# chrischoy/DeepGlobalRegistration

Measured on AMD Instinct MI355X. Metric: pair registrations/sec (FCGF x2 + 1-NN + 6-D inlier net + gate + weighted Procrustes + SE(3) refinement), higher is better.
Workload: dtype f32 results via 2 x f16 split operands (3 f16 MFMA products per MAC, f32 accumulate); k = 1 convs, kNN re-evaluation and registration in exact f32, SVD in f64

## Files before the change

### deepglobalregistration_amd/_lib.py

```python
import ctypes as C
import os
import threading

import torch

_HERE = os.path.dirname(os.path.abspath(__file__))
LIB_PATH = os.environ.get('DGR_HIP_LIB') or os.path.join(_HERE, 'lib', 'libdgr_hip.so')

DGR_OK, DGR_EINVAL, DGR_EHIP, DGR_ENOMEM, DGR_ESVD, DGR_EINTERNAL = 0, -1, -2, -3, -4, -5
STATUS_OK, STATUS_LOW_CONFIDENCE, STATUS_SVD_FAILED, STATUS_SAFEGUARD = 0, 1, 2, 3
STATUS_FLAG_ICP_SKIPPED, STATUS_MASK = 0x100, 0xff

c_i32p, c_i64p, c_f32p, c_f64p = (C.POINTER(C.c_int32), C.POINTER(C.c_int64),
                                  C.POINTER(C.c_float), C.POINTER(C.c_double))
vp = C.c_void_p


class WeightDesc(C.Structure):
    _fields_ = [('name', C.c_char_p), ('data', vp), ('numel', C.c_int64)]


class Params(C.Structure):
    _fields_ = [('clip_weight_thresh', C.c_float), ('voxel_size', C.c_float),
                ('inlier_feature_type', C.c_int), ('max_iter', C.c_int),
# ... 26 lines not shown
    'dgr_net_get_intermediate': (C.c_int, [vp, vp, C.c_char_p, vp, C.c_int64, c_i64p, c_i64p]),
    'dgr_net_layer_stats': (C.c_int, [vp, vp, C.c_int, c_i64p]),
    'dgr_net_num_layers': (C.c_int, [vp]),
    'dgr_net_rerun_layer': (C.c_int, [vp, vp, C.c_int, C.c_int, c_f32p, c_f32p]),
    'dgr_maps_create': (C.c_int, [vp, vp, C.c_int64, C.c_int, C.c_int, C.POINTER(vp), vp]),
    'dgr_maps_destroy': (None, [vp]),
    'dgr_maps_get_coords': (C.c_int, [vp, C.c_int, vp, C.c_int64, c_i64p]),
    'dgr_maps_get_kernel_map': (C.c_int, [vp, C.c_int, C.c_int, vp, C.c_int64, vp, vp, C.c_int64,
                                          c_i64p, c_i64p]),
    'dgr_knn1_l2': (C.c_int, [vp, vp, C.c_int64, vp, C.c_int64, C.c_int, C.c_int, vp, vp, vp]),
    'dgr_knn1_l2_batch': (C.c_int, [vp, vp, c_i64p, vp, c_i64p, C.c_int, C.c_int, C.c_int, vp, vp, vp]),
    'dgr_knn_l2': (C.c_int, [vp, vp, C.c_int64, vp, C.c_int64, C.c_int, C.c_int, C.c_int, vp, vp, vp]),
    'dgr_knn_l2_batch': (C.c_int, [vp, vp, c_i64p, vp, c_i64p, C.c_int, C.c_int, C.c_int, C.c_int, vp, vp,
                                   vp]),
    'dgr_inlier_inputs': (C.c_int, [vp, vp, vp, C.c_int64, vp, vp, C.c_int64, vp, C.c_int, vp, vp, vp]),
    'dgr_sigmoid_clip_sum': (C.c_int, [vp, vp, C.c_int64, C.c_float, vp, c_f64p, vp]),
    'dgr_gather_rows3': (C.c_int, [vp, vp, vp, C.c_int64, vp, vp]),
    'dgr_weighted_procrustes': (C.c_int, [vp, vp, vp, vp, C.c_int64, C.c_float, c_f32p, c_f32p, vp]),
    'dgr_se3_refine': (C.c_int, [vp, vp, vp, vp, C.c_int64, C.c_float, C.c_int, C.c_int, C.c_double,
                                 c_f32p, c_f32p, c_i32p, c_f32p, c_i32p, vp]),
    'dgr_register_batch': (C.c_int, [vp, vp, vp, vp, vp, c_i64p, vp, vp, c_i64p, C.c_int,
                                     C.POINTER(Params), vp, vp, c_f32p, c_i32p, c_f32p, vp]),
    'dgr_register_pairs': (C.c_int, [vp, vp, vp, vp, vp, c_i64p, C.c_int, C.c_int, c_i32p, C.c_int,
                                     C.POINTER(Params), vp, vp, c_f32p, c_i32p, c_f32p, vp]),
    'dgr_register_batch_f64': (C.c_int, [vp, c_f64p, C.c_int64, c_i64p]),
    'dgr_register_batch_output': (C.c_int, [vp, C.c_int, vp, C.c_int64, c_i64p, vp]),
    'dgr_ctx_set_profiling': (C.c_int, [vp, C.c_int]),
    'dgr_icp_point_to_point': (C.c_int, [vp, vp, C.c_int64, vp, C.c_int64, C.c_double, c_f64p, C.c_int, C.c_double,
                                          C.c_double, c_f64p, c_f64p, vp]),
    'dgr_ransac_correspondence': (C.c_int, [vp, vp, vp, C.c_int64, C.c_double, C.c_int64, C.c_uint32, c_f64p, c_f64p, vp]),
    'dgr_ctx_stage_times': (C.c_int, [vp, c_f32p]),
    'dgr_ctx_stage_times_v2': (C.c_int, [vp, c_f32p, C.c_int, C.POINTER(C.c_int)]),
    'dgr_ctx_conv_launches': (C.c_int64, [vp]),
    'dgr_ctx_conv_launch_times': (C.c_int, [vp, c_f32p, c_f32p, C.c_int64, C.POINTER(C.c_int64)]),
    'dgr_ctx_conv_launch_kernel_us': (C.c_int, [vp, c_f32p, C.c_int64, C.POINTER(C.c_int64)]),
    'dgr_ctx_conv_launch_kinds': (C.c_int, [vp, C.c_char_p, C.c_int64, C.POINTER(C.c_int64)]),
    'dgr_radius_pairs_batch': (C.c_int, [vp, vp, c_i64p, vp, c_i64p, C.c_int, c_f64p, C.c_double, C.c_int, vp, vp,
                                         C.c_int64, c_i64p, vp]),
    'dgr_pairs_isin_batch': (C.c_int, [vp, vp, c_i64p, vp, c_i64p, C.c_int, c_i64p, vp, vp]),
    'dgr_validation_counts': (C.c_int, [vp, vp, vp, C.c_float, c_i64p, C.c_int, c_i64p, vp]),
    'dgr_score_pairs': (C.c_int, [vp, vp, c_i64p, C.c_int, c_i32p, C.c_int, c_f64p, C.c_double, c_f64p, vp]),
    'dgr_pose_graph_optimize': (C.c_int, [vp, C.c_int, c_i64p, c_i64p, c_i32p, c_f64p, c_f64p, C.POINTER(C.c_uint8), c_f64p,
                                          C.POINTER(PgParams), c_f64p, c_f64p, c_f64p, vp]),
    'dgr_voxel_mean': (C.c_int, [vp, vp, C.c_int, c_i64p, C.c_int, c_i32p, C.c_int, c_f64p, c_f64p, C.c_double, vp, vp, vp, vp,
                                 vp, c_i64p, c_i64p, vp]),
    'dgr_tsdf_fragment': (C.c_int, [vp, vp, C.c_int, C.c_int, C.c_int, c_f64p, c_f64p, c_f64p, C.c_double, C.c_double,
                                    C.c_double, C.c_double, C.c_int, C.c_int, C.c_int, vp, C.c_int64, vp, vp, vp, C.c_int64,
                                    c_i64p, c_i64p, c_i64p, vp]),
    'dgr_debug_ortho2rotation': (C.c_int, [vp, vp, C.c_int64, vp, vp, vp, vp]),
    'dgr_debug_se3_refine_from': (C.c_int, [vp, vp, vp, vp, C.c_int64, C.c_float, C.c_int, C.c_int, C.c_double,
                                            c_f64p, c_f64p, vp]),
    'dgr_debug_smooth_l1': (C.c_int, [vp, vp, vp, C.c_int64, C.c_float, vp, vp]),
    'dgr_debug_conv_layer': (C.c_int, [vp, vp, C.c_int, vp, vp, C.c_int, C.c_int64, vp, vp]),
}

_lib = None


def load():
    global _lib
    if _lib is not None:
        return _lib
    if not os.path.exists(LIB_PATH):
        raise RuntimeError(
            f'{LIB_PATH} not found: the HIP extension is not built.  Run '
            '`python -c "import __graft_entry__ as g; g.build()"` (or `make -C '
            'deepglobalregistration_amd/csrc`).  There is no CPU fallback.')
    lib = C.CDLL(LIB_PATH)
    for name, (res, args) in SIGNATURES.items():
        fn = getattr(lib, name)
        fn.restype = res
        fn.argtypes = args
    _lib = lib
    return lib


class DgrError(RuntimeError):
    def __init__(self, code, message):
        super().__init__(f'libdgr_hip error {code}: {message}')
        self.code = code


class DgrInvalidArgument(DgrError, ValueError):

    def __init__(self, message):
        RuntimeError.__init__(self, f'libdgr_hip: {message}')
        self.code = DGR_EINVAL


def check(rc):
    if rc == DGR_OK:
        return
    msg = load().dgr_last_error().decode('utf-8', 'replace')
    if rc == DGR_EINVAL:
        raise DgrInvalidArgument(msg)
    raise DgrError(rc, msg)


_ctxs = {}
_tls = threading.local()


def new_ctx(device):
    lib = load()
    device = torch.device(device)
    idx = device.index if device.index is not None else torch.cuda.current_device()
# ... 40 lines not shown
```

### deepglobalregistration_amd/csrc/conv.hip

```cpp
#include <stdlib.h>

#include <map>

#include "dgr_internal.h"
#include <algorithm>
#include "hash.h"
#include "split.h"

typedef float f32x16 __attribute__((ext_vector_type(16)));
typedef float f32x4 __attribute__((ext_vector_type(4)));
typedef _Float16 f16x4 __attribute__((ext_vector_type(4)));
typedef int i32x4 __attribute__((ext_vector_type(4)));
typedef unsigned int u32x2 __attribute__((ext_vector_type(2)));
typedef unsigned int u32x4 __attribute__((ext_vector_type(4)));

struct ConvKArgs {
  const float *in;
  float *out;
  float *y;
  const float *shift;
  const float *w;
  const int32_t *pair_in, *pair_out, *tile_ptr, *rule_ptr, *n_rows_dev;
  const int4 *tile_desc;
  int in_ld, out_ld, in_relu, y_ld;
// ... 355 lines not shown

template <int CP, int NBLK>
static int launch_identity(const ConvKArgs &ka, int64_t rows_cap, int num_cus, hipStream_t stream) {
  int64_t blocks = std::min<int64_t>((int64_t)num_cus * 4, std::max<int64_t>(1, dgr_ceil_div(rows_cap, 32 * 4 * 2)));
  identity_conv_kernel<CP, NBLK><<<(int)blocks, 256, 0, stream>>>(ka);
  DGR_LAUNCH_CHECK();
  return DGR_OK;
}

int dgr_conv_launch(const DgrConvLaunch &a, int num_cus, hipStream_t stream, const char **kernel_name) {
  ConvKArgs ka;
  ka.in = a.in; ka.out = a.out; ka.w = a.w; ka.y = a.y; ka.shift = a.shift; ka.y_ld = a.cout;
  ka.pair_in = a.pair_in; ka.pair_out = a.pair_out; ka.tile_ptr = a.tile_ptr; ka.rule_ptr = a.rule_ptr;
  ka.n_rows_dev = a.n_rows_dev; ka.tile_desc = a.tile_desc;
  ka.in_ld = a.in_ld; ka.out_ld = a.out_ld; ka.in_relu = a.in_relu;
  ka.cin = a.cin; ka.cin_pad = a.cin_pad; ka.cout = a.cout; ka.K = a.K;
  ka.l2_normalize = a.l2_normalize;
  DGR_REQUIRE(!a.l2_normalize || (a.pair_in == nullptr && a.cout <= 32 && a.cout_pad == 32),
              "fused l2 normalisation needs an identity map and Cout <= 32 (got %d)", a.cout);
  DGR_REQUIRE(a.cin_pad % 8 == 0 && a.cin_pad >= a.cin && a.cin_pad <= 256, "bad cin_pad %d", a.cin_pad);
  const int64_t tile_bound = a.tile_bound > 0 ? a.tile_bound : (int64_t)num_cus * 4;
  const bool vec = ((a.cin | a.in_ld) & 3) == 0;
  if (a.pair_in == nullptr && vec && a.cin == a.cin_pad && a.tile_bound > 0) {
#define DGR_ID(CPV, NBV)                                                                          \
  if (a.cin_pad == CPV && a.cout_pad == 32 * NBV) {                                               \
    if (kernel_name) *kernel_name = "identity_conv_kernel<" #CPV ", " #NBV ">";                   \
    return launch_identity<CPV, NBV>(ka, a.tile_bound * DGR_TILE_M, num_cus, stream);             \
  }
    DGR_ID(64, 1) DGR_ID(64, 2) DGR_ID(96, 2)
#undef DGR_ID
  }
#define DGR_V2(CPV, WMV, WNV, MBV, NBV)                                                                        \
  if (a.cin_pad == CPV) {                                                                                       \
    if (kernel_name)                                                                                            \
      *kernel_name = vec ? "sparse_conv_mfma_v2<" #CPV ", " #WMV ", " #WNV ", " #MBV ", " #NBV ", true>"        \
                         : "sparse_conv_mfma_v2<" #CPV ", " #WMV ", " #WNV ", " #MBV ", " #NBV ", false>";      \
    return vec ? launch_v2<CPV, WMV, WNV, MBV, NBV, true>(ka, tile_bound, num_cus, stream)                     \
               : launch_v2<CPV, WMV, WNV, MBV, NBV, false>(ka, tile_bound, num_cus, stream);                   \
  }
  switch (a.cout_pad) {
    case 32: DGR_V2(8, 2, 1, 1, 1) DGR_V2(32, 2, 1, 1, 1) DGR_V2(64, 2, 1, 1, 1) break;
    case 64: DGR_V2(32, 2, 2, 1, 1) DGR_V2(64, 2, 2, 1, 1) DGR_V2(96, 2, 2, 1, 1) DGR_V2(128, 2, 2, 1, 1)
             DGR_V2(256, 2, 2, 1, 1) break;
    case 128: DGR_V2(64, 1, 4, 2, 1) DGR_V2(128, 1, 4, 2, 1) DGR_V2(256, 1, 4, 2, 1) break;
    case 256: DGR_V2(128, 1, 4, 2, 2) DGR_V2(256, 1, 4, 2, 2) break;
    default: break;
  }
#undef DGR_V2
  dgr_set_error("sparse conv: no kernel instantiation for Cin (padded) %d -> Cout (padded) %d", a.cin_pad, a.cout_pad);
  return DGR_EINVAL;
}

template <int LPR, bool SPLIT>
__global__ void __launch_bounds__(256)
    reduce_rows_kernel(const float *__restrict__ y, int y_ld, const int32_t *__restrict__ ptr,
                       const int32_t *__restrict__ pos, const int32_t *n_dev, float *__restrict__ out, int out_ld,
                       const float *__restrict__ shift, const float *__restrict__ res, int res_ld, int res_relu,
                       unsigned char *__restrict__ planes, float *__restrict__ scale_out, int out_relu) {
  constexpr int ROWS = 256 / LPR;
  const int n = *n_dev;
  const int sub = threadIdx.x / LPR, c = (threadIdx.x % LPR) * 4;
  for (int64_t row = (int64_t)blockIdx.x * ROWS + sub; row < n; row += (int64_t)gridDim.x * ROWS) {
    f32x4 acc = shift ? *reinterpret_cast<const f32x4 *>(shift + c) : f32x4{0.f, 0.f, 0.f, 0.f};
    if (res) {
      f32x4 r = *reinterpret_cast<const f32x4 *>(res + row * res_ld + c);
      if (res_relu) { r.x = fmaxf(r.x, 0.f); r.y = fmaxf(r.y, 0.f); r.z = fmaxf(r.z, 0.f); r.w = fmaxf(r.w, 0.f); }
      acc += r;
    }
    int j = ptr[row];
    const int end = ptr[row + 1];
    for (; j + 8 <= end; j += 8) {
      int p[8];
#pragma unroll
      for (int u = 0; u < 8; ++u) p[u] = pos[j + u];
      f32x4 v[8];
#pragma unroll
      for (int u = 0; u < 8; ++u) v[u] = dgr_y_load<LPR == 64>(y + (int64_t)p[u] * y_ld + c);
#pragma unroll
      for (int u = 0; u < 8; ++u) acc += v[u];
    }
    for (; j + 4 <= end; j += 4) {
      const int p0 = pos[j], p1 = pos[j + 1], p2 = pos[j + 2], p3 = pos[j + 3];
      const f32x4 v0 = dgr_y_load<LPR == 64>(y + (int64_t)p0 * y_ld + c);
      const f32x4 v1 = dgr_y_load<LPR == 64>(y + (int64_t)p1 * y_ld + c);
      const f32x4 v2 = dgr_y_load<LPR == 64>(y + (int64_t)p2 * y_ld + c);
      const f32x4 v3 = dgr_y_load<LPR == 64>(y + (int64_t)p3 * y_ld + c);
      acc += v0; acc += v1; acc += v2; acc += v3;
    }
    for (; j < end; ++j) acc += dgr_y_load<LPR == 64>(y + (int64_t)pos[j] * y_ld + c);
    if (!SPLIT || out) *reinterpret_cast<f32x4 *>(out + row * out_ld + c) = acc;
    if constexpr (SPLIT) {
      const int lo = out_relu ? 0 : (int)0x80000000;
      const i32x4 ab = __builtin_bit_cast(i32x4, acc);
      int xb[4];
      uint32_t mx = 0;
#pragma unroll
      for (int u = 0; u < 4; ++u) {
        xb[u] = max(ab[u], lo);
        mx = max(mx, (uint32_t)xb[u] & 0x7fffffffu);
      }
#pragma unroll
      for (int d = LPR / 2; d >= 1; d >>= 1) mx = max(mx, (uint32_t)__shfl_xor((int)mx, d, 64));
      const float sx = dgr_row_scale_of(mx);
      f16x4 h, m;
#pragma unroll
      for (int u = 0; u < 4; ++u) {
        _Float16 hh, mm;
        dgr_split2(__builtin_bit_cast(float, xb[u]), sx, hh, mm);
        h[u] = hh; m[u] = mm;
      }
      const bool odd = threadIdx.x & 1;
      const u32x2 hb = __builtin_bit_cast(u32x2, h), mb = __builtin_bit_cast(u32x2, m);
      const u32x2 give = odd ? hb : mb;
      u32x2 got;
      got.x = (uint32_t)__shfl_xor((int)give.x, 1, 64);
      got.y = (uint32_t)__shfl_xor((int)give.y, 1, 64);
      const u32x4 st = odd ? u32x4{got.x, got.y, mb.x, mb.y} : u32x4{hb.x, hb.y, got.x, got.y};
      unsigned char *dst = planes + row * (LPR * 16);
      *reinterpret_cast<u32x4 *>(dst + dgr_split_row_offset(c & ~7, odd ? 1 : 0)) = st;
      if (c == 0) scale_out[row] = sx;
    }
  }
}

int dgr_reduce_rows(const float *y, int cout, const int32_t *ptr, const int32_t *pos, const int32_t *n_dev,
                    int64_t n_cap, float *out, int out_ld, const float *shift, const float *res, int res_ld,
                    int res_relu, hipStream_t stream, const DgrSplitRows *split, int out_relu) {
  DGR_REQUIRE((out_ld & 3) == 0 && (res == nullptr || (res_ld & 3) == 0), "reduce_rows: row strides must be x4");
  DGR_REQUIRE(out || split, "reduce_rows: no output");
  DGR_REQUIRE(!split || (split->planes && split->scale && split->channels == cout && cout % 64 == 0),
              "reduce_rows: split rows need planes, scales and the layer's width (a multiple of 64)");
  const int lpr = cout / 4;
  const int64_t want = std::max<int64_t>(1, dgr_ceil_div(n_cap, 256 / lpr));
#define DGR_RR1(L, SP)                                                                                         \
  do {                                                                                                         \
    static int resident = 0;                                                                                   \
    if (resident == 0) {                                                                                       \
      int per_cu = 0, dev = 0, cus = 0;                                                                        \
      DGR_HIP_CHECK(hipOccupancyMaxActiveBlocksPerMultiprocessor(&per_cu, reduce_rows_kernel<L, SP>, 256, 0)); \
      DGR_HIP_CHECK(hipGetDevice(&dev));                                                                       \
      DGR_HIP_CHECK(hipDeviceGetAttribute(&cus, hipDeviceAttributeMultiprocessorCount, dev));                  \
      resident = (per_cu < 1 ? 1 : per_cu) * (cus < 1 ? 1 : cus);                                              \
    }                                                                                                          \
    const int64_t blocks = want > resident ? (int64_t)resident * std::min<int64_t>(4, want / resident) : want; \
    reduce_rows_kernel<L, SP><<<(int)blocks, 256, 0, stream>>>(y, cout, ptr, pos, n_dev, out, out_ld, shift,   \
                                                               res, res_ld, res_relu, split ? split->planes : nullptr, \
                                                               split ? split->scale : nullptr, out_relu);      \
  } while (0)
#define DGR_RR(L)                       \
  do {                                  \
    if (split) DGR_RR1(L, true);        \
    else DGR_RR1(L, false);             \
  } while (0)
  switch (cout) {
    case 32: DGR_RR1(8, false); break;
    case 64: DGR_RR(16); break;
    case 128: DGR_RR(32); break;
    case 256: DGR_RR(64); break;
    default:
      dgr_set_error("reduce_rows: unsupported width %d", cout);
      return DGR_EINVAL;
  }
#undef DGR_RR1
#undef DGR_RR
  DGR_LAUNCH_CHECK();
  return DGR_OK;
}

__global__ void __launch_bounds__(256)
    conv_small_cin_kernel(const float *__restrict__ in, int in_ld, int in_relu, int cin,
                          const float *__restrict__ w, const float *__restrict__ shift,
                          const int32_t *__restrict__ out_ptr, const int32_t *__restrict__ out_pos,
                          const int32_t *__restrict__ pair_in, const uint16_t *__restrict__ pair_k,
                          const int32_t *n_out_dev, float *__restrict__ out, int out_ld) {
  const int n = *n_out_dev;
  const int co = threadIdx.x & 31;
  for (int64_t o = (int64_t)blockIdx.x * 8 + (threadIdx.x >> 5); o < n; o += (int64_t)gridDim.x * 8) {
    float acc = shift ? shift[co] : 0.f;
    const int end = out_ptr[o + 1];
    int j = out_ptr[o];
    for (; j + 8 <= end; j += 8) {
      int pos[8], row[8], kk[8];
#pragma unroll
      for (int u = 0; u < 8; ++u) pos[u] = out_pos[j + u];
#pragma unroll
      for (int u = 0; u < 8; ++u) { row[u] = pair_in[pos[u]]; kk[u] = pair_k[pos[u]]; }
      float y[8];
#pragma unroll
      for (int u = 0; u < 8; ++u) {
        const float *wk = w + (int64_t)kk[u] * 256;
        float t = 0.f;
        for (int ci = 0; ci < cin; ++ci) {
          float x = in[(int64_t)row[u] * in_ld + ci];
          if (in_relu) x = fmaxf(x, 0.f);
          t = fmaf(x, wk[(32 * (ci >> 2) + co) * 4 + (ci & 3)], t);
        }
        y[u] = t;
      }
#pragma unroll
      for (int u = 0; u < 8; ++u) acc += y[u];
    }
    for (; j < end; ++j) {
      const int pos = out_pos[j];
      const int row = pair_in[pos];
      const float *wk = w + (int64_t)pair_k[pos] * 256;
      float y = 0.f;
      for (int ci = 0; ci < cin; ++ci) {
        float x = in[(int64_t)row * in_ld + ci];
        if (in_relu) x = fmaxf(x, 0.f);
        y = fmaf(x, wk[(32 * (ci >> 2) + co) * 4 + (ci & 3)], y);
      }
      acc += y;
    }
    out[o * out_ld + co] = acc;
  }
}

template <int CIN>
__global__ void __launch_bounds__(256)
// ... 569 lines not shown
```

### deepglobalregistration_amd/csrc/dgr_internal.h

```cpp
#pragma once
#include <hip/hip_runtime.h>
#include <stdint.h>
#include <stdio.h>
#include <stdlib.h>
#include <string>
#include <vector>

#include "../../include/dgr_hip.h"

void dgr_set_error(const char *fmt, ...);

#define DGR_HIP_CHECK(expr)                                                                  \
  do {                                                                                       \
    hipError_t _e = (expr);                                                                  \
    if (_e != hipSuccess) {                                                                  \
      dgr_set_error("%s:%d: %s failed: %s", __FILE__, __LINE__, #expr, hipGetErrorString(_e)); \
      return DGR_EHIP;                                                                       \
    }                                                                                        \
  } while (0)

#define DGR_CHECK(expr)          \
  do {                           \
    int _r = (expr);             \
    if (_r != DGR_OK) return _r; \
// ... 105 lines not shown
  DgrKernelMap down[3];
  int32_t *overflow = nullptr;
};

int dgr_build_maps(DgrArena &arena, const int32_t *coords, int64_t N, int D, int conv1_ks,
                   DgrMapSet *ms, hipStream_t stream, bool skip_conv1_map = false, bool lean = false,
                   bool nbr_tables = false);
int dgr_nbr_counts(const DgrNbrTable &t, const int32_t *n_out_dev, int64_t counts[27]);
int dgr_conv1_probe(DgrArena &arena, const DgrCoordMap &cm, int ks, const float *in, int in_ld, int cin,
                    const float *w_tiled, const float *shift, float *out, int out_ld, int32_t *pair_count,
                    hipStream_t stream, const float *w_compact = nullptr, const char **kernel_name = nullptr,
                    uint32_t *out_amax = nullptr);
int dgr_unique_rows(DgrArena &arena, const int32_t *keys, int64_t n, int nc, int32_t *first_flag,
                    int32_t *rank, int32_t *n_unique_dev, int32_t **table_out, uint32_t *mask_out,
                    hipStream_t stream);
int dgr_exclusive_scan_i32(DgrArena &arena, const int32_t *in, int32_t *out, int64_t n,
                           int32_t *total_out, hipStream_t stream);
constexpr int DGR_SCAN_MAX = 24;
int dgr_exclusive_scan_multi(DgrArena &arena, int count, const int32_t *const *in, int32_t *const *out, const int64_t *n,
                             int32_t *const *total_out, hipStream_t stream);

struct DgrConvLaunch {
  const float *in;
  int in_ld;
  int in_relu;
  float *out;
  int out_ld;
  float *y;
  const float *shift;
  const float *w;
  int cin, cin_pad, cout, cout_pad, K;
  const int32_t *pair_in, *pair_out, *tile_ptr, *rule_ptr;
  const int4 *tile_desc;
  const int32_t *n_rows_dev;
  int64_t tile_bound;
  int l2_normalize = 0;
  unsigned long long *clk = nullptr;
};
int dgr_conv_launch(const DgrConvLaunch &a, int num_cus, hipStream_t stream, const char **kernel_name = nullptr);
struct DgrSplitRows {
  unsigned char *planes = nullptr;
  float *scale = nullptr;
  int channels = 0;
};
bool dgr_conv_wide_supported(int cin_pad, int cin, int cout);
int dgr_conv_wide_launch(const DgrConvLaunch &a, const DgrSplitRows &in, const void *wb, int64_t piece_stride,
                         float w_unscale, int num_cus, hipStream_t stream, const char **kernel_name = nullptr);
int dgr_row_amax(const float *in, int in_ld, int cin, int relu, const int32_t *n_dev, int64_t n_cap, uint32_t *out,
                 hipStream_t stream);
int dgr_split_rows(const float *in, int in_ld, int relu, const int32_t *n_dev, int64_t n_cap, const DgrSplitRows &out,
                   hipStream_t stream);
int dgr_reduce_rows(const float *y, int cout, const int32_t *ptr, const int32_t *pos, const int32_t *n_dev,
                    int64_t n_cap, float *out, int out_ld, const float *shift, const float *res, int res_ld,
                    int res_relu, hipStream_t stream, const DgrSplitRows *split = nullptr, int out_relu = 0);
int dgr_conv_small_cin(const float *in, int in_ld, int in_relu, int cin, const float *w_tiled, const float *w_quad,
                       const float *shift, const DgrKernelMap &km, const int32_t *n_out_dev, int64_t n_out_cap, float *out,
                       int out_ld, hipStream_t stream);
struct DgrConvOsLaunch {
  const float *in; int in_ld, in_relu;
  float *out; int out_ld, out_relu;
  const float *w16, *shift;
  const void *wb3; int64_t piece_stride;
  const void *wbd = nullptr;
  const uint32_t *row_amax = nullptr; float w_unscale = 1.f;
  uint32_t *out_amax = nullptr, *out_amax2 = nullptr;
  int64_t n_in_cap = 0;
  const float *res; int res_ld, res_relu;
  int rows_per_block;
  int phase_channels = 64;
  const DgrNbrTable *nbr;
  const int32_t *n_out_dev;
  int64_t n_out_cap;
  int cin, cin_pad, cout;
  bool dense = false;
  bool up = false;
  const unsigned char *in_dsplit = nullptr;
  unsigned char *out_dsplit = nullptr;
};
int dgr_conv_os_launch(const DgrConvOsLaunch &a, hipStream_t stream, const char **kernel_name = nullptr);
bool dgr_conv_dense_supported(int cin, int cin_pad, int cout);
int dgr_conv_dense_launch(const DgrConvOsLaunch &a, hipStream_t stream, const char **kernel_name = nullptr);
bool dgr_conv_up_supported(int cin, int cin_pad, int cout);
int dgr_conv_up_launch(const DgrConvOsLaunch &a, hipStream_t stream, const char **kernel_name = nullptr);
int dgr_l2_normalize_rows(const float *in, int in_ld, float *out, int out_ld, int c, int relu,
                          const int32_t *n_dev, int64_t n_cap, hipStream_t stream);

struct DgrBatchOutputs {
  const void *ptr[5] = {nullptr, nullptr, nullptr, nullptr, nullptr};
  int64_t numel[5] = {0, 0, 0, 0, 0};
  uint64_t generation = 0;
};

struct DgrEventPool {
  std::vector<hipEvent_t> ev;
  size_t used = 0;
  hipEvent_t next();
  void release();
};

struct dgr_ctx {
  int device = 0;
  int num_cus = 256;
  DgrArena arena;
  bool profiling = false;
  float stage_ms[9] = {0, 0, 0, 0, 0, 0, 0, 0, 0};
  int64_t conv_launches = 0;
  DgrBatchOutputs last;
// ... 74 lines not shown
```

### deepglobalregistration_amd/csrc/net.hip

```cpp
#include <math.h>
#include <stdlib.h>
#include <string.h>

#include <algorithm>
#include <map>
#include <memory>
#include <string>

#include "dgr_internal.h"

static const int CH[5] = {0, 32, 64, 128, 256};
static const int TR[5] = {0, 64, 64, 64, 128};
static constexpr float BN_EPS = 1e-5f;

struct DgrLayer {
  std::string name;
  int K, cin, cout, cin_pad, cout_pad;
  float *w = nullptr;
  float *w16 = nullptr;
  void *w16b = nullptr;
  void *w16d = nullptr;
  int64_t w16b_piece = 0;
  float *wc = nullptr;
  float *wq = nullptr;
// ... 486 lines not shown
      for (int l = 0; l < 4; ++l) same_stride = same_stride || t == &ms.nsame[l];
      o.dense = same_stride && o.row_amax && o.wbd && !os_lists && dgr_conv_dense_supported(L.cin, L.cin_pad, L.cout) &&
                cin_map.n_cap * (int64_t)in.ld * 4 < (1ll << 31);
      DGR_REQUIRE(o.dense || (!in.dsplit_only && !out.dsplit_only), "layer %s: dense split rows outside the dense-tile kernel", L.name.c_str());
      static const bool no_up = getenv("DGR_NO_UP") != nullptr;
      o.up = swapped && !o.dense && !no_up && !os_lists && o.row_amax && o.wbd && t->perm && res == nullptr &&
             dgr_conv_up_supported(L.cin, L.cin_pad, L.cout) && cin_map.n_cap * (int64_t)in.ld * 4 < (1ll << 31);
      if (o.dense) {
        o.in_dsplit = in.dsplit;
        o.out_dsplit = out.dsplit;
        if (out.dsplit_only) o.out = nullptr;
      }
      const char *kname = "sparse_conv_os";
      DGR_CHECK(dgr_conv_os_launch(o, stream, &kname));
      if (prof) {
        DGR_HIP_CHECK(hipEventRecord(e1, stream));
        ctx->conv_spans.push_back({e0, e1});
        ctx->gemm_spans.push_back({e0, e1});
        ctx->conv_kinds.push_back(kname);
      }
      LayerRun &r = net->runs[li];
      r = LayerRun();
      r.os = true;
      r.os_launch = o;
      r.nbr = *t;
      r.os_launch.nbr = &r.nbr;
      r.n_in = cin_map.n_dev; r.n_out = cout_map.n_dev; r.K = L.K;
      r.n_out_cap = cout_map.n_cap;
      return DGR_OK;
    }
    const bool small_cin = km && !swapped && !res && L.cin <= 8 && L.cout == 32 && L.cin_pad == 8;
    const char *kname = (L.cin == 6 && L.wq) ? "conv_cin6_quad_kernel" : L.cin == 1 ? "conv_small_cin_row_kernel" : "conv_small_cin_kernel";
    unsigned long long *clk = nullptr;
    const bool wide = L.wb && km;
    if (small_cin)
      DGR_CHECK(dgr_conv_small_cin(in.ptr, in.ld, in.relu, L.cin, L.w, L.wq, L.shift, *km, cout_map.n_dev, cout_map.n_cap,
                                   out.ptr, out.ld, stream));
    else if (wide) {
      DGR_REQUIRE(in.split.planes, "layer %s: the wide-layer kernel needs its input as split rows", L.name.c_str());
      if (prof) {
        DGR_ALLOC(a.clk, ctx->arena, unsigned long long, 2);
        DGR_HIP_CHECK(hipMemsetAsync(a.clk, 0xff, sizeof(unsigned long long), stream));
        DGR_HIP_CHECK(hipMemsetAsync(a.clk + 1, 0, sizeof(unsigned long long), stream));
        clk = a.clk;
      }
      DGR_CHECK(dgr_conv_wide_launch(a, in.split, L.wb, L.wb_piece, L.w_unscale, ctx->num_cus, stream, &kname));
    } else
      DGR_CHECK(dgr_conv_launch(a, ctx->num_cus, stream, &kname));
    if (prof) DGR_HIP_CHECK(hipEventRecord(em, stream));
    DGR_REQUIRE(!out.split.planes || (km && !small_cin), "layer %s: only a reduction can write split rows", L.name.c_str());
    if (km && !small_cin)
      DGR_CHECK(dgr_reduce_rows(ybuf, L.cout, swapped ? km->in_ptr : km->out_ptr, swapped ? km->in_pos : km->out_pos,
                                cout_map.n_dev, cout_map.n_cap, out.split_only ? nullptr : out.ptr, out.ld, L.shift, res ? res->ptr : nullptr,
                                res ? res->ld : 0, res ? res->relu : 0, stream, out.split.planes ? &out.split : nullptr,
                                out.relu));
    if (prof) {
      DGR_HIP_CHECK(hipEventRecord(e1, stream));
      ctx->conv_spans.push_back({e0, e1});
      ctx->gemm_spans.push_back({e0, em});
      ctx->conv_kinds.push_back(kname);
      ctx->conv_clks.resize(ctx->conv_spans.size(), nullptr);
      ctx->conv_clks.back() = clk;
    }
    LayerRun &r = net->runs[li];
    a.clk = nullptr;
    r.launch = a;
    r.split_in = wide ? in.split : DgrSplitRows();
    r.split_out = out.split;
    r.out_relu = out.relu;
    r.split_only = out.split_only;
    r.has_reduce = km != nullptr;
    r.small_cin = small_cin;
    if (km) r.km = *km;
    if (km) {
      r.red_ptr = swapped ? km->in_ptr : km->out_ptr;
      r.red_pos = swapped ? km->in_pos : km->out_pos;
    }
    r.n_out_cap = cout_map.n_cap;
    r.res = res ? res->ptr : nullptr; r.res_ld = res ? res->ld : 0; r.res_relu = res ? res->relu : 0;
    r.rule_ptr = km ? km->rule_ptr : nullptr;
    r.n_in = cin_map.n_dev; r.n_out = cout_map.n_dev; r.K = L.K;
    return DGR_OK;
  }
};

int dgr_resunet_forward_impl(dgr_ctx *ctx, dgr_net *net, const int32_t *coords, const float *feats,
                             int64_t N, float *out, hipStream_t stream) {
  DgrArena &A = ctx->arena;
  Fwd f;
  f.ctx = ctx; f.net = net; f.stream = stream; f.prof = ctx->profiling;
  hipEvent_t m0 = nullptr, m1 = nullptr;
  if (f.prof) {
    m0 = ctx->events.next(); m1 = ctx->events.next();
    DGR_HIP_CHECK(hipEventRecord(m0, stream));
  }
  f.ms.overflow = ctx->flag_dev;
  const bool use_nbr = net->D == 3 && net->cin <= 8 && net->conv1_ks <= 7;
  const bool conv1_fused = use_nbr;
  DGR_CHECK(dgr_build_maps(A, coords, N, net->D, net->conv1_ks, &f.ms, stream, conv1_fused, true, use_nbr));
  if (f.prof) {
    DGR_HIP_CHECK(hipEventRecord(m1, stream));
    (net->D == 3 ? ctx->map3_spans : ctx->map6_spans).push_back({m0, m1});
  }
  {
    const DgrMapSet &m = f.ms;
    int64_t need = m.use_nbr ? 64 : m.conv1.pair_cap * 32;
    const int64_t same_c[4] = {64, 64, 128, 256}, down_c[3] = {64, 128, 256};
// ... 326 lines not shown
  int32_t n_in = 0, n_out = 0;
  DGR_HIP_CHECK(hipMemcpy(&n_in, r.n_in, sizeof(int32_t), hipMemcpyDeviceToHost));
  DGR_HIP_CHECK(hipMemcpy(&n_out, r.n_out, sizeof(int32_t), hipMemcpyDeviceToHost));
  int64_t P = n_out, kne = 1;
  if (r.os) {
    int64_t counts[27];
    DGR_CHECK(dgr_nbr_counts(r.nbr, r.n_out, counts));
    P = 0;
    kne = 0;
    for (int k = 0; k < 27; ++k) { P += counts[k]; kne += counts[k] > 0; }
  } else if (r.fused_pairs) {
    int32_t pc = 0;
    DGR_HIP_CHECK(hipMemcpy(&pc, r.fused_pairs, sizeof(int32_t), hipMemcpyDeviceToHost));
    P = pc;
    kne = r.K;
  } else if (r.rule_ptr) {
    std::vector<int32_t> rp(r.K + 1);
    DGR_HIP_CHECK(hipMemcpy(rp.data(), r.rule_ptr, (size_t)(r.K + 1) * sizeof(int32_t), hipMemcpyDeviceToHost));
    P = rp[r.K];
    kne = 0;
    for (int k = 0; k < r.K; ++k) kne += rp[k + 1] > rp[k];
  }
  stats[0] = P; stats[1] = kne; stats[2] = n_in; stats[3] = n_out;
  stats[4] = L.cin; stats[5] = L.cout; stats[6] = L.K; stats[7] = 0;
  return DGR_OK;
}

extern "C" int dgr_net_rerun_layer(dgr_ctx *ctx, dgr_net *net, int layer, int reps, float *gemm_ms, float *reduce_ms) {
  DGR_REQUIRE(ctx && net && gemm_ms && reduce_ms && reps > 0, "bad argument");
  DGR_REQUIRE(layer >= 0 && layer < (int)net->W->layers.size(), "layer %d out of range", layer);
  const LayerRun &r = net->runs[layer];
  DGR_REQUIRE(r.n_in && r.n_out, "run a forward first");
  DGR_REQUIRE(net->run_generation == ctx->arena.generation,
              "the kernel maps of the last forward are gone: a later call on this context reused its workspace");
  DGR_REQUIRE(!r.fused_pairs, "layer %d ran fused with its neighbour search; not re-runnable", layer);
  const DgrLayer &L = net->W->layers[layer];
  hipEvent_t e0, e1, e2;
  DGR_HIP_CHECK(hipEventCreate(&e0)); DGR_HIP_CHECK(hipEventCreate(&e1)); DGR_HIP_CHECK(hipEventCreate(&e2));
  float tg = 0.f, tr = 0.f;
  for (int i = 0; i < reps + 1; ++i) {
    DGR_HIP_CHECK(hipEventRecord(e0, nullptr));
    if (r.os)
      DGR_CHECK(dgr_conv_os_launch(r.os_launch, nullptr));
    else if (r.small_cin)
      DGR_CHECK(dgr_conv_small_cin(r.launch.in, r.launch.in_ld, r.launch.in_relu, L.cin, L.w, L.wq, L.shift, r.km, r.n_out,
                                   r.n_out_cap, r.launch.out, r.launch.out_ld, nullptr));
    else if (L.wb && r.has_reduce)
      DGR_CHECK(dgr_conv_wide_launch(r.launch, r.split_in, L.wb, L.wb_piece, L.w_unscale, ctx->num_cus, nullptr));
    else
      DGR_CHECK(dgr_conv_launch(r.launch, ctx->num_cus, nullptr));
    DGR_HIP_CHECK(hipEventRecord(e1, nullptr));
    if (r.has_reduce && !r.small_cin && !r.os)
      DGR_CHECK(dgr_reduce_rows(r.launch.y, L.cout, r.red_ptr, r.red_pos, r.n_out, r.n_out_cap,
                                r.split_only ? nullptr : r.launch.out, r.launch.out_ld, L.shift, r.res, r.res_ld, r.res_relu, nullptr,
                                r.split_out.planes ? &r.split_out : nullptr, r.out_relu));
    DGR_HIP_CHECK(hipEventRecord(e2, nullptr));
    DGR_HIP_CHECK(hipEventSynchronize(e2));
    float a = 0.f, b = 0.f;
    DGR_HIP_CHECK(hipEventElapsedTime(&a, e0, e1));
    DGR_HIP_CHECK(hipEventElapsedTime(&b, e1, e2));
    if (i > 0) { tg += a; tr += b; }
  }
  (void)hipEventDestroy(e0); (void)hipEventDestroy(e1); (void)hipEventDestroy(e2);
  *gemm_ms = tg / reps;
  *reduce_ms = tr / reps;
  return DGR_OK;
}
```

### deepglobalregistration_amd/ops.py

```python
import ctypes as C

import numpy as np
import torch

from . import _lib
from ._lib import check, get_ctx, ptr, stream_ptr, vp

F32_EPS = float(np.finfo(np.float32).eps)


def _dev(t):
    if not (torch.is_tensor(t) and t.is_cuda):
        raise ValueError('expected a CUDA(ROCm) tensor')
    return t.device


def _as(t, dtype, device):
    if not torch.is_tensor(t):
        t = torch.as_tensor(np.asarray(t))
    return t.to(device=device, dtype=dtype).contiguous()


def voxelize(xyz, voxel_size, batch_index=0, device='cuda'):
    lib = _lib.load()
# ... 943 lines not shown
    n = C.c_int(0)
    check(_lib.load().dgr_ctx_stage_times_v2(get_ctx(device), t, 16, C.byref(n)))
    names = ['fcgf', 'knn', 'inlier_inputs', 'inlier_net', 'registration', 'maps_3d', 'maps_6d', 'conv_kernels', 'o3d_steps']
    out = dict(zip(names, [float(v) for v in t[:n.value]]))
    out['conv_launches'] = int(_lib.load().dgr_ctx_conv_launches(get_ctx(device)))
    return out


def conv_launch_times(device):
    cap = 4096
    t, g = (C.c_float * cap)(), (C.c_float * cap)()
    n = C.c_int64(0)
    check(_lib.load().dgr_ctx_conv_launch_times(get_ctx(device), t, g, cap, C.byref(n)))
    return [float(t[i]) for i in range(n.value)], [float(g[i]) for i in range(n.value)]


def conv_launch_kernel_us(device):
    cap = 4096
    t = (C.c_float * cap)()
    n = C.c_int64(0)
    check(_lib.load().dgr_ctx_conv_launch_kernel_us(get_ctx(device), t, cap, C.byref(n)))
    return [float(t[i]) for i in range(n.value)]


def conv_launch_kinds(device):
    cap = 1 << 16
    buf = C.create_string_buffer(cap)
    n = C.c_int64(0)
    check(_lib.load().dgr_ctx_conv_launch_kinds(get_ctx(device), buf, cap, C.byref(n)))
    names = buf.value.decode().split('\n')
    return names[:n.value]


def debug_ortho2rotation(p6, grad_R=None):
    dev = _dev(p6)
    p6 = _as(p6, torch.float32, dev).reshape(-1, 6)
    n = p6.shape[0]
    R = torch.empty((n, 3, 3), dtype=torch.float32, device=dev)
    g = dp = None
    if grad_R is not None:
        g = _as(grad_R, torch.float32, dev).reshape(n, 9)
        dp = torch.empty((n, 6), dtype=torch.float32, device=dev)
    check(_lib.load().dgr_debug_ortho2rotation(get_ctx(dev), ptr(p6), n, ptr(g), ptr(R), ptr(dp), stream_ptr(dev.index)))
    return (R, dp) if grad_R is not None else R


def debug_smooth_l1(X, Y, quantization_size):
    dev = _dev(X)
    X, Y = _as(X, torch.float32, dev), _as(Y, torch.float32, dev)
    out = torch.empty(X.shape[0], dtype=torch.float32, device=dev)
    check(_lib.load().dgr_debug_smooth_l1(get_ctx(dev), ptr(X), ptr(Y), X.shape[0], float(quantization_size), ptr(out),
                                          stream_ptr(dev.index)))
    return out
```

### include/dgr_hip.h

```cpp
#ifndef DGR_HIP_H
#define DGR_HIP_H

#include <stdint.h>

#ifdef __cplusplus
extern "C" {
#endif

typedef struct dgr_ctx dgr_ctx;
typedef struct dgr_net dgr_net;
typedef struct dgr_maps dgr_maps;
typedef void *dgr_stream;

enum {
  DGR_OK = 0,
  DGR_EINVAL = -1,
  DGR_EHIP = -2,
  DGR_ENOMEM = -3,
  DGR_ESVD = -4,
  DGR_EINTERNAL = -5
};

enum { DGR_STATUS_OK = 0, DGR_STATUS_LOW_CONFIDENCE = 1, DGR_STATUS_SVD_FAILED = 2,
       DGR_STATUS_SAFEGUARD = 3 ,
// ... 126 lines not shown
int dgr_ctx_conv_launch_kinds(dgr_ctx *ctx, char *buf, int64_t capacity, int64_t *n);

int dgr_radius_pairs_batch(dgr_ctx *ctx, const float *xyz0, const int64_t *off0, const float *xyz1,
                           const int64_t *off1, int npairs, const double *T, double radius, int K,
                           int32_t *counts_out, int64_t *pairs_out, int64_t capacity, int64_t *total_out,
                           dgr_stream stream);
int dgr_pairs_isin_batch(dgr_ctx *ctx, const int64_t *pos, const int64_t *pos_off, const int64_t *pred,
                         const int64_t *pred_off, int npairs, const int64_t *M_per_pair, uint8_t *out,
                         dgr_stream stream);
int dgr_validation_counts(dgr_ctx *ctx, const uint8_t *label, const float *weights, float threshold,
                          const int64_t *off, int npairs, int64_t *counts_out, dgr_stream stream);

#define DGR_SCORE_WIDTH 11
int dgr_score_pairs(dgr_ctx *ctx, const float *bank_xyz, const int64_t *bank_off, int nfrag, const int32_t *pair_ids,
                    int npairs, const double *T, double radius, double *sums_out, dgr_stream stream);

#define DGR_PG_MAX_NODES 128
typedef struct {
  double mu;
  int reference_node;
  int max_iter;
  double rel_tol;
} dgr_pg_params;
int dgr_pose_graph_optimize(dgr_ctx *ctx, int ngraphs, const int64_t *node_off, const int64_t *edge_off,
                            const int32_t *edge_ids, const double *edge_T, const double *edge_info,
                            const uint8_t *edge_uncertain, const double *pose_init, const dgr_pg_params *params,
                            double *pose_out, double *line_out, double *stats_out, dgr_stream stream);

#define DGR_VM_FRAC_BITS 40
int dgr_voxel_mean(dgr_ctx *ctx, const void *xyz, int is_f64, const int64_t *off, int nfrag, const int32_t *frag_ids,
                   int nsel, const double *T, const double *origin, double voxel_size, int64_t *first_out,
                   int32_t *coords_out, int32_t *count_out, int64_t *fsum_out, double *mean_out, int64_t *n_out,
                   int64_t *dropped_out, dgr_stream stream);

#define DGR_TSDF_BLOCK_LIMIT 67108864
int dgr_tsdf_fragment(dgr_ctx *ctx, const uint16_t *depth, int nframes, int height, int width, const double *intrinsic,
                      const double *pose, const double *extrinsic, double voxel_length, double sdf_trunc,
                      double depth_scale, double depth_trunc, int block, int stride, int min_weight, double *xyz_out,
                      int64_t max_points, int32_t *blocks_out, float *tsdf_out, int32_t *weight_out, int64_t max_blocks,
                      int64_t *n_blocks_out, int64_t *n_points_out, int64_t *kept_out, dgr_stream stream);

int dgr_debug_ortho2rotation(dgr_ctx *ctx, const float *p6, int64_t n, const float *grad_R9, float *R9_out,
                             float *grad_p6_out, dgr_stream stream);
int dgr_debug_se3_refine_from(dgr_ctx *ctx, const float *X, const float *Y, const float *w, int64_t N,
                              float quantization_size, int max_iter, int max_break_count,
                              double break_threshold_ratio, const double *state_in, double *state_out,
                              dgr_stream stream);
int dgr_debug_smooth_l1(dgr_ctx *ctx, const float *X, const float *Y, int64_t n, float quantization_size,
                        float *per_point_out, dgr_stream stream);

int dgr_debug_conv_layer(dgr_ctx *ctx, dgr_net *net, int layer, const int32_t *coords, const float *in, int in_relu,
                         int64_t N, float *out, dgr_stream stream);

#ifdef __cplusplus
}
#endif
#endif
```

Measured before the change: 390.5.

## Add software-pipelined gather-reduce kernel for sparse conv row reduction

Adds a new reduce_rows_pipe_kernel that becomes the default for the post-GEMM scatter-reduce. It prefetches row ranges, gather indices and residuals for the next grid-stride iterations and issues the first gathers for the next row before finishing the current one. Indices are loaded cooperatively once per lane and broadcast with readlane/shuffle instead of each lane reading pos separately. The goal is to hide gather latency. The cost is more registers, more complex control flow, and predicated dummy loads for empty rows. The old kernel stays available through an environment variable, and a debug entry point is added.

Measured after the change: 391.3, median of 6. No clear change (+0.2%).

```diff
diff --git a/deepglobalregistration_amd/_lib.py b/deepglobalregistration_amd/_lib.py
--- a/deepglobalregistration_amd/_lib.py
+++ b/deepglobalregistration_amd/_lib.py
@@ -102,6 +102,8 @@
                                             c_f64p, c_f64p, vp]),
     'dgr_debug_smooth_l1': (C.c_int, [vp, vp, vp, C.c_int64, C.c_float, vp, vp]),
     'dgr_debug_conv_layer': (C.c_int, [vp, vp, C.c_int, vp, vp, C.c_int, C.c_int64, vp, vp]),
+    'dgr_debug_reduce_rows': (C.c_int, [vp, C.c_int, vp, C.c_int, vp, vp, vp, C.c_int64, vp, vp, C.c_int, C.c_int, vp,
+                                        C.c_int, vp, vp, C.c_int, C.c_int, vp]),
 }
 
 _lib = None
diff --git a/deepglobalregistration_amd/csrc/conv.hip b/deepglobalregistration_amd/csrc/conv.hip
--- a/deepglobalregistration_amd/csrc/conv.hip
+++ b/deepglobalregistration_amd/csrc/conv.hip
@@ -431,6 +431,44 @@
 }
 
 template <int LPR, bool SPLIT>
+__device__ __forceinline__ void reduce_rows_finish(const f32x4 acc, int64_t row, int c, float *__restrict__ out,
+                                                   int out_ld, unsigned char *__restrict__ planes,
+                                                   float *__restrict__ scale_out, int out_relu) {
+  if (!SPLIT || out) *reinterpret_cast<f32x4 *>(out + row * out_ld + c) = acc;
+  if constexpr (SPLIT) {
+    const int lo = out_relu ? 0 : (int)0x80000000;
+    const i32x4 ab = __builtin_bit_cast(i32x4, acc);
+    int xb[4];
+    uint32_t mx = 0;
+#pragma unroll
+    for (int u = 0; u < 4; ++u) {
+      xb[u] = max(ab[u], lo);
+      mx = max(mx, (uint32_t)xb[u] & 0x7fffffffu);
+    }
+#pragma unroll
+    for (int d = LPR / 2; d >= 1; d >>= 1) mx = max(mx, (uint32_t)__shfl_xor((int)mx, d, 64));
+    const float sx = dgr_row_scale_of(mx);
+    f16x4 h, m;
+#pragma unroll
+    for (int u = 0; u < 4; ++u) {
+      _Float16 hh, mm;
+      dgr_split2(__builtin_bit_cast(float, xb[u]), sx, hh, mm);
+      h[u] = hh; m[u] = mm;
+    }
+    const bool odd = threadIdx.x & 1;
+    const u32x2 hb = __builtin_bit_cast(u32x2, h), mb = __builtin_bit_cast(u32x2, m);
+    const u32x2 give = odd ? hb : mb;
+    u32x2 got;
+    got.x = (uint32_t)__shfl_xor((int)give.x, 1, 64);
+    got.y = (uint32_t)__shfl_xor((int)give.y, 1, 64);
+    const u32x4 st = odd ? u32x4{got.x, got.y, mb.x, mb.y} : u32x4{hb.x, hb.y, got.x, got.y};
+    unsigned char *dst = planes + row * (LPR * 16);
+    *reinterpret_cast<u32x4 *>(dst + dgr_split_row_offset(c & ~7, odd ? 1 : 0)) = st;
+    if (c == 0) scale_out[row] = sx;
+  }
+}
+
+template <int LPR, bool SPLIT>
 __global__ void __launch_bounds__(256)
     reduce_rows_kernel(const float *__restrict__ y, int y_ld, const int32_t *__restrict__ ptr,
                        const int32_t *__restrict__ pos, const int32_t *n_dev, float *__restrict__ out, int out_ld,
@@ -467,64 +505,162 @@
       acc += v0; acc += v1; acc += v2; acc += v3;
     }
     for (; j < end; ++j) acc += dgr_y_load<LPR == 64>(y + (int64_t)pos[j] * y_ld + c);
-    if (!SPLIT || out) *reinterpret_cast<f32x4 *>(out + row * out_ld + c) = acc;
-    if constexpr (SPLIT) {
-      const int lo = out_relu ? 0 : (int)0x80000000;
-      const i32x4 ab = __builtin_bit_cast(i32x4, acc);
-      int xb[4];
-      uint32_t mx = 0;
-#pragma unroll
-      for (int u = 0; u < 4; ++u) {
-        xb[u] = max(ab[u], lo);
-        mx = max(mx, (uint32_t)xb[u] & 0x7fffffffu);
-      }
-#pragma unroll
-      for (int d = LPR / 2; d >= 1; d >>= 1) mx = max(mx, (uint32_t)__shfl_xor((int)mx, d, 64));
-      const float sx = dgr_row_scale_of(mx);
-      f16x4 h, m;
-#pragma unroll
-      for (int u = 0; u < 4; ++u) {
-        _Float16 hh, mm;
-        dgr_split2(__builtin_bit_cast(float, xb[u]), sx, hh, mm);
-        h[u] = hh; m[u] = mm;
-      }
-      const bool odd = threadIdx.x & 1;
-      const u32x2 hb = __builtin_bit_cast(u32x2, h), mb = __builtin_bit_cast(u32x2, m);
-      const u32x2 give = odd ? hb : mb;
-      u32x2 got;
-      got.x = (uint32_t)__shfl_xor((int)give.x, 1, 64);
-      got.y = (uint32_t)__shfl_xor((int)give.y, 1, 64);
-      const u32x4 st = odd ? u32x4{got.x, got.y, mb.x, mb.y} : u32x4{hb.x, hb.y, got.x, got.y};
-      unsigned char *dst = planes + row * (LPR * 16);
-      *reinterpret_cast<u32x4 *>(dst + dgr_split_row_offset(c & ~7, odd ? 1 : 0)) = st;
-      if (c == 0) scale_out[row] = sx;
-    }
-  }
-}
-
-int dgr_reduce_rows(const float *y, int cout, const int32_t *ptr, const int32_t *pos, const int32_t *n_dev,
-                    int64_t n_cap, float *out, int out_ld, const float *shift, const float *res, int res_ld,
-                    int res_relu, hipStream_t stream, const DgrSplitRows *split, int out_relu) {
+    reduce_rows_finish<LPR, SPLIT>(acc, row, c, out, out_ld, planes, scale_out, out_relu);
+  }
+}
+
+template <int LPR>
+__device__ __forceinline__ const float *reduce_rows_src(const float *__restrict__ y, int y_ld, int c, int g0, int cur,
+                                                        int cnt, const float *idle, int k) {
+  const int kk = min(k, cnt - 1);
+  int p;
+  if constexpr (LPR == 64) p = __builtin_amdgcn_readlane(cur, kk & 63);
+  else p = __shfl(cur, g0 + max(kk, 0), 64);
+  return cnt > 0 ? y + (int64_t)p * y_ld : idle;
+}
+template <int LPR, int DD>
+__device__ __forceinline__ void reduce_rows_request(f32x4 (&v)[DD], const float *__restrict__ y, int y_ld, int c, int g0,
+                                                    int cur, int cnt, const float *idle) {
+#pragma unroll
+  for (int u = 0; u < DD; ++u) v[u] = dgr_y_load<LPR == 64>(reduce_rows_src<LPR>(y, y_ld, c, g0, cur, cnt, idle, u) + c);
+}
+template <int LPR, int DD>
+__device__ __forceinline__ void reduce_rows_add(f32x4 &acc, f32x4 (&v)[DD], const float *__restrict__ y, int y_ld, int c,
+                                                int g0, int cur, int cnt, const float *idle) {
+  constexpr int R = LPR / DD;
+#pragma unroll
+  for (int rd = 0; rd < R; ++rd) {
+    const int u0 = rd * DD;
+    if (rd + 1 < R && __builtin_amdgcn_ballot_w64(u0 + DD < cnt) != 0) {
+#pragma unroll
+      for (int u = 0; u < DD; ++u) {
+        const f32x4 s = acc + v[u];
+        acc = u0 + u < cnt ? s : acc;
+        v[u] = dgr_y_load<LPR == 64>(reduce_rows_src<LPR>(y, y_ld, c, g0, cur, cnt, idle, u0 + DD + u) + c);
+      }
+    } else {
+#pragma unroll
+      for (int u = 0; u < DD; ++u) {
+        const f32x4 s = acc + v[u];
+        acc = u0 + u < cnt ? s : acc;
+      }
+      break;
+    }
+  }
+}
+
+template <int LPR, bool SPLIT>
+__global__ void __launch_bounds__(256)
+    reduce_rows_pipe_kernel(const float *__restrict__ y, int y_ld, const int32_t *__restrict__ ptr,
+                            const int32_t *__restrict__ pos, const int32_t *n_dev, float *__restrict__ out, int out_ld,
+                            const float *__restrict__ shift, const float *__restrict__ res, int res_ld, int res_relu,
+                            unsigned char *__restrict__ planes, float *__restrict__ scale_out, int out_relu) {
+  constexpr int ROWS = 256 / LPR, G = 64 / LPR, DD = LPR == 64 ? 8 : 4;
+  const int n = *n_dev;
+  const int lane = threadIdx.x & 63, t = threadIdx.x % LPR, c = t * 4, g0 = lane - t, gi = lane / LPR;
+  const int64_t step = (int64_t)gridDim.x * ROWS;
+  int64_t wrow = (int64_t)blockIdx.x * ROWS + __builtin_amdgcn_readfirstlane((int)(threadIdx.x >> 6)) * G;
+  if (wrow >= n) return;
+  auto range_of = [&](int64_t r, int &first, int &last) {
+    first = 0; last = 0;
+    if (r < n) { first = ptr[r]; last = ptr[r + 1]; }
+  };
+  auto indices_of = [&](int first, int last) -> int { return first + t < last ? pos[first + t] : 0; };
+  auto residual_of = [&](int64_t r) -> f32x4 {
+    if (res && r < n) return *reinterpret_cast<const f32x4 *>(res + r * res_ld + c);
+    return f32x4{0.f, 0.f, 0.f, 0.f};
+  };
+  auto count_of = [&](int pairs) -> int {
+    const int k = max(0, min(pairs, LPR));
+    if constexpr (LPR == 64) return __builtin_amdgcn_readfirstlane(k);
+    return k;
+  };
+  auto idle_of = [&](unsigned long long some, int idx, int64_t wr) -> const float * {
+    if (some) return y + (int64_t)__builtin_amdgcn_readlane(idx, (int)__builtin_ctzll(some)) * y_ld;
+    return out ? out + wr * out_ld : reinterpret_cast<const float *>(planes + wr * (LPR * 16));
+  };
+  auto moved = [](int x) -> int { return __builtin_amdgcn_mov_dpp(x, 0xE4, 0xF, 0xF, true); };
+  i32x4 shb = __builtin_bit_cast(i32x4, shift ? *reinterpret_cast<const f32x4 *>(shift + c) : f32x4{0.f, 0.f, 0.f, 0.f});
+  shb = i32x4{moved(shb.x), moved(shb.y), moved(shb.z), moved(shb.w)};
+  const f32x4 sh = __builtin_bit_cast(f32x4, shb);
+  int j0, end, nj0, nend, nnj0, nnend;
+  range_of(wrow + gi, j0, end);
+  int cur = indices_of(j0, end);
+  range_of(wrow + step + gi, nj0, nend);
+  int nidx = indices_of(nj0, nend);
+  range_of(wrow + 2 * step + gi, nnj0, nnend);
+  f32x4 r = residual_of(wrow + gi);
+  int cnt = count_of(end - j0);
+  const float *idle = idle_of(__builtin_amdgcn_ballot_w64(cnt > 0), cur, wrow);
+  f32x4 v[DD];
+  reduce_rows_request<LPR, DD>(v, y, y_ld, c, g0, cur, cnt, idle);
+  for (;;) {
+    const int64_t row = wrow + gi;
+    const bool valid = row < n;
+    f32x4 acc = sh;
+    if (res && valid) {
+      if (res_relu) { r.x = fmaxf(r.x, 0.f); r.y = fmaxf(r.y, 0.f); r.z = fmaxf(r.z, 0.f); r.w = fmaxf(r.w, 0.f); }
+      acc += r;
+    }
+    reduce_rows_add<LPR, DD>(acc, v, y, y_ld, c, g0, cur, cnt, idle);
+    for (int base = j0 + LPR; __builtin_amdgcn_ballot_w64(base < end) != 0; base += LPR) {
+      const int ci = indices_of(base, end);
+      const int cc = count_of(end - base);
+      const float *cs = idle_of(__builtin_amdgcn_ballot_w64(cc > 0), ci, wrow);
+      f32x4 w[DD];
+      reduce_rows_request<LPR, DD>(w, y, y_ld, c, g0, ci, cc, cs);
+      reduce_rows_add<LPR, DD>(acc, w, y, y_ld, c, g0, ci, cc, cs);
+    }
+    const bool again = wrow + step < n;
+    if (again) {
+      j0 = moved(nj0); end = moved(nend); cur = moved(nidx); nj0 = moved(nnj0); nend = moved(nnend);
+      nidx = indices_of(nj0, nend);
+      range_of(wrow + 3 * step + gi, nnj0, nnend);
+      r = residual_of(wrow + step + gi);
+      cnt = count_of(end - j0);
+      idle = idle_of(__builtin_amdgcn_ballot_w64(cnt > 0), cur, wrow + step);
+      reduce_rows_request<LPR, DD>(v, y, y_ld, c, g0, cur, cnt, idle);
+    }
+    if (valid) reduce_rows_finish<LPR, SPLIT>(acc, row, c, out, out_ld, planes, scale_out, out_relu);
+    if (!again) break;
+    wrow += step;
+  }
+}
+
+static int reduce_rows_launch(int variant, const float *y, int cout, const int32_t *ptr, const int32_t *pos,
+                              const int32_t *n_dev, int64_t n_cap, float *out, int out_ld, const float *shift,
+                              const float *res, int res_ld, int res_relu, int num_cus, hipStream_t stream,
+                              const DgrSplitRows *split, int out_relu) {
   DGR_REQUIRE((out_ld & 3) == 0 && (res == nullptr || (res_ld & 3) == 0), "reduce_rows: row strides must be x4");
   DGR_REQUIRE(out || split, "reduce_rows: no output");
   DGR_REQUIRE(!split || (split->planes && split->scale && split->channels == cout && cout % 64 == 0),
               "reduce_rows: split rows need planes, scales and the layer's width (a multiple of 64)");
+  if (num_cus <= 0) {
+    int dev = 0;
+    DGR_HIP_CHECK(hipGetDevice(&dev));
+    DGR_HIP_CHECK(hipDeviceGetAttribute(&num_cus, hipDeviceAttributeMultiprocessorCount, dev));
+    if (num_cus < 1) num_cus = 1;
+  }
   const int lpr = cout / 4;
   const int64_t want = std::max<int64_t>(1, dgr_ceil_div(n_cap, 256 / lpr));
-#define DGR_RR1(L, SP)                                                                                         \
+#define DGR_RR2(KERNEL, L, SP)                                                                                 \
   do {                                                                                                         \
-    static int resident = 0;                                                                                   \
-    if (resident == 0) {                                                                                       \
-      int per_cu = 0, dev = 0, cus = 0;                                                                        \
-      DGR_HIP_CHECK(hipOccupancyMaxActiveBlocksPerMultiprocessor(&per_cu, reduce_rows_kernel<L, SP>, 256, 0)); \
-      DGR_HIP_CHECK(hipGetDevice(&dev));                                                                       \
-      DGR_HIP_CHECK(hipDeviceGetAttribute(&cus, hipDeviceAttributeMultiprocessorCount, dev));                  \
-      resident = (per_cu < 1 ? 1 : per_cu) * (cus < 1 ? 1 : cus);                                              \
+    static int per_cu = 0;                                                                                     \
+    if (per_cu == 0) {                                                                                         \
+      int q = 0;                                                                                               \
+      DGR_HIP_CHECK(hipOccupancyMaxActiveBlocksPerMultiprocessor(&q, KERNEL<L, SP>, 256, 0));                  \
+      per_cu = q < 1 ? 1 : q;                                                                                  \
     }                                                                                                          \
-    const int64_t blocks = want > resident ? (int64_t)resident * std::min<int64_t>(4, want / resident) : want; \
-    reduce_rows_kernel<L, SP><<<(int)blocks, 256, 0, stream>>>(y, cout, ptr, pos, n_dev, out, out_ld, shift,   \
-                                                               res, res_ld, res_relu, split ? split->planes : nullptr, \
-                                                               split ? split->scale : nullptr, out_relu);      \
+    const int64_t resident = (int64_t)per_cu * num_cus;                                                        \
+    const int64_t blocks = want > resident ? resident * std::min<int64_t>(4, want / resident) : want;          \
+    KERNEL<L, SP><<<(int)blocks, 256, 0, stream>>>(y, cout, ptr, pos, n_dev, out, out_ld, shift, res, res_ld,  \
+                                                   res_relu, split ? split->planes : nullptr,                  \
+                                                   split ? split->scale : nullptr, out_relu);                  \
+  } while (0)
+#define DGR_RR1(L, SP)                                         \
+  do {                                                         \
+    if (variant == 1) DGR_RR2(reduce_rows_kernel, L, SP);      \
+    else DGR_RR2(reduce_rows_pipe_kernel, L, SP);              \
   } while (0)
 #define DGR_RR(L)                       \
   do {                                  \
@@ -540,10 +676,33 @@
       dgr_set_error("reduce_rows: unsupported width %d", cout);
       return DGR_EINVAL;
   }
+#undef DGR_RR2
 #undef DGR_RR1
 #undef DGR_RR
   DGR_LAUNCH_CHECK();
   return DGR_OK;
+}
+
+int dgr_reduce_rows(const float *y, int cout, const int32_t *ptr, const int32_t *pos, const int32_t *n_dev,
+                    int64_t n_cap, float *out, int out_ld, const float *shift, const float *res, int res_ld,
+                    int res_relu, int num_cus, hipStream_t stream, const DgrSplitRows *split, int out_relu) {
+  static const bool v1 = getenv("DGR_REDUCE_V1") != nullptr;
+  return reduce_rows_launch(v1 ? 1 : 2, y, cout, ptr, pos, n_dev, n_cap, out, out_ld, shift, res, res_ld, res_relu,
+                            num_cus, stream, split, out_relu);
+}
+
+extern "C" int dgr_debug_reduce_rows(dgr_ctx *ctx, int variant, const float *y, int width, const int32_t *ptr,
+                                     const int32_t *pos, const int32_t *n_dev, int64_t n_cap, const float *shift,
+                                     const float *res, int res_ld, int res_relu, float *out, int out_ld,
+                                     unsigned char *planes, float *scales, int out_relu, int num_cus,
+                                     dgr_stream stream) {
+  DGR_REQUIRE(ctx && y && ptr && n_dev && n_cap > 0, "dgr_debug_reduce_rows: bad argument");
+  DGR_REQUIRE(variant == 1 || variant == 2, "dgr_debug_reduce_rows: variant %d is neither 1 nor 2", variant);
+  DGR_REQUIRE((planes == nullptr) == (scales == nullptr), "dgr_debug_reduce_rows: planes and scales come together");
+  DgrSplitRows split;
+  split.planes = planes; split.scale = scales; split.channels = width;
+  return reduce_rows_launch(variant, y, width, ptr, pos, n_dev, n_cap, out, out_ld, shift, res, res_ld, res_relu, num_cus,
+                            (hipStream_t)stream, planes ? &split : nullptr, out_relu);
 }
 
 __global__ void __launch_bounds__(256)
diff --git a/deepglobalregistration_amd/csrc/dgr_internal.h b/deepglobalregistration_amd/csrc/dgr_internal.h
--- a/deepglobalregistration_amd/csrc/dgr_internal.h
+++ b/deepglobalregistration_amd/csrc/dgr_internal.h
@@ -181,7 +181,7 @@
                    hipStream_t stream);
 int dgr_reduce_rows(const float *y, int cout, const int32_t *ptr, const int32_t *pos, const int32_t *n_dev,
                     int64_t n_cap, float *out, int out_ld, const float *shift, const float *res, int res_ld,
-                    int res_relu, hipStream_t stream, const DgrSplitRows *split = nullptr, int out_relu = 0);
+                    int res_relu, int num_cus, hipStream_t stream, const DgrSplitRows *split = nullptr, int out_relu = 0);
 int dgr_conv_small_cin(const float *in, int in_ld, int in_relu, int cin, const float *w_tiled, const float *w_quad,
                        const float *shift, const DgrKernelMap &km, const int32_t *n_out_dev, int64_t n_out_cap, float *out,
                        int out_ld, hipStream_t stream);
diff --git a/deepglobalregistration_amd/csrc/net.hip b/deepglobalregistration_amd/csrc/net.hip
--- a/deepglobalregistration_amd/csrc/net.hip
+++ b/deepglobalregistration_amd/csrc/net.hip
@@ -562,7 +562,7 @@
     if (km && !small_cin)
       DGR_CHECK(dgr_reduce_rows(ybuf, L.cout, swapped ? km->in_ptr : km->out_ptr, swapped ? km->in_pos : km->out_pos,
                                 cout_map.n_dev, cout_map.n_cap, out.split_only ? nullptr : out.ptr, out.ld, L.shift, res ? res->ptr : nullptr,
-                                res ? res->ld : 0, res ? res->relu : 0, stream, out.split.planes ? &out.split : nullptr,
+                                res ? res->ld : 0, res ? res->relu : 0, ctx->num_cus, stream, out.split.planes ? &out.split : nullptr,
                                 out.relu));
     if (prof) {
       DGR_HIP_CHECK(hipEventRecord(e1, stream));
@@ -995,8 +995,8 @@
     DGR_HIP_CHECK(hipEventRecord(e1, nullptr));
     if (r.has_reduce && !r.small_cin && !r.os)
       DGR_CHECK(dgr_reduce_rows(r.launch.y, L.cout, r.red_ptr, r.red_pos, r.n_out, r.n_out_cap,
-                                r.split_only ? nullptr : r.launch.out, r.launch.out_ld, L.shift, r.res, r.res_ld, r.res_relu, nullptr,
-                                r.split_out.planes ? &r.split_out : nullptr, r.out_relu));
+                                r.split_only ? nullptr : r.launch.out, r.launch.out_ld, L.shift, r.res, r.res_ld, r.res_relu, ctx->num_cus,
+                                nullptr, r.split_out.planes ? &r.split_out : nullptr, r.out_relu));
     DGR_HIP_CHECK(hipEventRecord(e2, nullptr));
     DGR_HIP_CHECK(hipEventSynchronize(e2));
     float a = 0.f, b = 0.f;
diff --git a/deepglobalregistration_amd/ops.py b/deepglobalregistration_amd/ops.py
--- a/deepglobalregistration_amd/ops.py
+++ b/deepglobalregistration_amd/ops.py
@@ -1019,3 +1019,20 @@
     check(_lib.load().dgr_debug_smooth_l1(get_ctx(dev), ptr(X), ptr(Y), X.shape[0], float(quantization_size), ptr(out),
                                           stream_ptr(dev.index)))
     return out
+
+
+def debug_reduce_rows(y, ptr_rows, pos, n_dev, n_cap, shift=None, res=None, res_relu=False, out=None, planes=None,
+                      scales=None, out_relu=False, variant=2, num_cus=0):
+    dev = _dev(y)
+    width = y.shape[1]
+    for t, dt in ((y, torch.float32), (ptr_rows, torch.int32), (pos, torch.int32), (n_dev, torch.int32),
+                  (shift, torch.float32), (res, torch.float32), (out, torch.float32), (planes, torch.uint8),
+                  (scales, torch.float32)):
+        assert t is None or (t.dtype == dt and t.is_contiguous() and t.device == y.device), 'debug_reduce_rows: bad tensor'
+    assert out is None or (out.shape[0] >= n_cap and out.shape[1] == width)
+    assert planes is None or (planes.shape[0] >= n_cap and planes.shape[1] == 4 * width and scales.shape[0] >= n_cap)
+    assert res is None or res.shape[1] == width
+    check(_lib.load().dgr_debug_reduce_rows(get_ctx(dev), int(variant), ptr(y), int(width), ptr(ptr_rows), ptr(pos), ptr(n_dev),
+                                            int(n_cap), ptr(shift), ptr(res), width if res is not None else 0,
+                                            int(bool(res_relu)), ptr(out), width, ptr(planes), ptr(scales),
+                                            int(bool(out_relu)), int(num_cus), stream_ptr(dev.index)))
diff --git a/include/dgr_hip.h b/include/dgr_hip.h
--- a/include/dgr_hip.h
+++ b/include/dgr_hip.h
@@ -202,6 +202,11 @@
 int dgr_debug_conv_layer(dgr_ctx *ctx, dgr_net *net, int layer, const int32_t *coords, const float *in, int in_relu,
                          int64_t N, float *out, dgr_stream stream);
 
+int dgr_debug_reduce_rows(dgr_ctx *ctx, int variant, const float *y, int width, const int32_t *ptr, const int32_t *pos,
+                          const int32_t *n_dev, int64_t n_cap, const float *shift, const float *res, int res_ld,
+                          int res_relu, float *out, int out_ld, unsigned char *planes, float *scales, int out_relu,
+                          int num_cus, dgr_stream stream);
+
 #ifdef __cplusplus
 }
 #endif
```
